# elisabeth96/nerf-rs

Hardware: AMD Instinct MI355X
Metric: rays/sec, lego 800x800 (64 coarse + 128 fine samples per ray) (higher is better)
Workload: dtype f32

## Files before the change

nerf-rs_amd/csrc/mlp_f32_core.hip.h:

```cpp
#pragma once
#include <hip/hip_runtime.h>
#include <stdint.h>

#include "mlp_common.hip.h"
#include "mlp_layout.h"

#ifndef NERF_DIAG_NO_BARRIER
#define NERF_DIAG_NO_BARRIER 0
#endif
#ifndef NERF_DIAG_NO_DMA
#define NERF_DIAG_NO_DMA 0
#endif
#ifndef NERF_DIAG_NO_LDS
#define NERF_DIAG_NO_LDS 0
#endif

namespace mlpf32 {

using namespace nerfmlp;
using namespace mlpdev;

constexpr int kReluGroup = 16;
constexpr int kLdsGroup = 1;

struct Pipe {
    const LDS_AS char *rd_base;
    const LDS_AS char *ring_lane;
    uint32_t rd_slot_off;
    f32x4 nx[2 * kLdsGroup];
    f32x4 cu[2 * kLdsGroup];
    uint32_t ring_addr;
    uint32_t wr_slot_off;
    uint32_t next_off;
    uint32_t stream_bytes;
    const char *gbase;
    const char *cur_src;
    uint32_t cur_dst;
    uint32_t lane16;
    uint64_t zs_off;
    uint32_t zs_exec;
    uint32_t zs_total;
};

__device__ __forceinline__ void pipe_zskip_init(Pipe &P, int zero_skip) {
    P.zs_off = zero_skip ? 0ull : ~0ull;
    P.zs_exec = 0;
    P.zs_total = 0;
}

__device__ __forceinline__ void pipe_zskip_report(const Pipe &P, unsigned long long *stats, int lane) {
    if (stats && lane == 0) {
        atomicAdd(stats, (unsigned long long)P.zs_exec);
        atomicAdd(stats + 1, (unsigned long long)P.zs_total);
    }
}

__device__ __forceinline__ void pipe_next_chunk(Pipe &P) {
    uint32_t off = P.next_off, slot = P.wr_slot_off;
    asm volatile("" : "+s"(off), "+s"(slot));
    P.cur_src = P.gbase + off;
    P.cur_dst = P.ring_addr + slot;
    off += kChunkBytes;
    P.next_off = (off == P.stream_bytes) ? 0u : off;
    slot += kChunkBytes;
    P.wr_slot_off = (slot == kRingSlots * kChunkBytes) ? 0u : slot;
    dma_set_dst(P.cur_dst);
}

__device__ __forceinline__ void pipe_issue_piece(Pipe &P, int i) {
#if !NERF_DIAG_NO_DMA
    glds_piece_m0(P.lane16, P.cur_src, i);
#else
    (void)P; (void)i;
#endif
}

__device__ __forceinline__ void pipe_issue(Pipe &P) {
    pipe_next_chunk(P);
#pragma unroll
    for (int i = 0; i < 4; ++i) pipe_issue_piece(P, i);
}

__device__ __forceinline__ void pipe_sync(Pipe &P) {
#if NERF_DIAG_NO_BARRIER
    asm volatile("s_waitcnt vmcnt(%0)" ::"n"(4 * (kRingSlots - 3)) : "memory");
#else
    asm volatile("s_waitcnt vmcnt(%0)\n\ts_barrier" ::"n"(4 * (kRingSlots - 3)) : "memory");
#endif
    pipe_next_chunk(P);
}

__device__ __forceinline__ void pipe_mid_step(Pipe &P, int ms) {
    if (ms >= 4) {
        __builtin_amdgcn_sched_barrier(0);
        pipe_issue_piece(P, ms - 4);
        __builtin_amdgcn_sched_barrier(0);
    }
}

__device__ __forceinline__ void pipe_prime(Pipe &P) {
#pragma unroll
    for (int j = 0; j < kLdsGroup; ++j) {
        P.nx[2 * j] = *(const LDS_AS f32x4 *)(P.rd_base + j * 2048);
        P.nx[2 * j + 1] = *(const LDS_AS f32x4 *)(P.rd_base + j * 2048 + 1024);
    }
}

__device__ __forceinline__ void pipe_restart(Pipe &P) {
    asm volatile("s_waitcnt vmcnt(0)\n\ts_barrier" ::: "memory");
    P.next_off = 0;
    P.wr_slot_off = 0;
#pragma unroll
    for (int c = 0; c < kRingSlots - 1; ++c) pipe_issue(P);
    asm volatile("s_waitcnt vmcnt(0)\n\ts_barrier" ::: "memory");
    P.rd_slot_off = 0;
    P.rd_base = P.ring_lane;
    pipe_prime(P);
}

__device__ __forceinline__ void pipe_advance(Pipe &P, int ms, f32x4 &a0, f32x4 &a1) {
    constexpr int LG = kLdsGroup;
    if (ms % LG == 0) {
#pragma unroll
        for (int j = 0; j < 2 * LG; ++j) P.cu[j] = P.nx[j];
        int nxt = ms + LG;
        if (nxt == 8) {
            uint32_t off = P.rd_slot_off + kChunkBytes;
            off = (off == kRingSlots * kChunkBytes) ? 0u : off;
            P.rd_slot_off = off;
            P.rd_base = P.ring_lane + off;
            nxt = 0;
        }
#pragma unroll
        for (int j = 0; j < LG; ++j) {
#if NERF_DIAG_NO_LDS
            asm volatile("" : "+v"(P.nx[2 * j]), "+v"(P.nx[2 * j + 1]));
#else
            P.nx[2 * j] = *(const LDS_AS f32x4 *)(P.rd_base + (nxt + j) * 2048);
            P.nx[2 * j + 1] = *(const LDS_AS f32x4 *)(P.rd_base + (nxt + j) * 2048 + 1024);
#endif
        }
        __builtin_amdgcn_sched_barrier(0);
    }
    a0 = P.cu[2 * (ms % LG)];
    a1 = P.cu[2 * (ms % LG) + 1];
}

#define MFMA(a, b, c) __builtin_amdgcn_mfma_f32_32x32x2f32((a), (b), (c), 0, 0, 0)

__device__ __forceinline__ uint64_t relu_live(float &b) {
    int bits = __builtin_bit_cast(int, b);
    asm volatile("" : "+v"(bits));
    b = __builtin_bit_cast(float, bits);
    return __builtin_amdgcn_ballot_w64(bits != 0);
}

template <int NT, bool RELU>
__device__ __forceinline__ void tile_steps(const f32x16 &in, f32x16 (&out)[NT], Pipe &P) {
    static_assert(NT == 8 || NT == 4, "NT");
    constexpr int G = RELU ? kReluGroup : 1;
    float bq[G];
    if constexpr (RELU) P.zs_total += 16;
    if constexpr (NT == 8) {
        uint64_t live[G];
#pragma unroll
        for (int r = 0; r < 16; ++r) {
            f32x4 a0, a1;
            if ((r & 7) == 4) pipe_sync(P);
            pipe_advance(P, r & 7, a0, a1);
            if (r % G == 0) {
#pragma unroll
                for (int g = 0; g < G; ++g) bq[g] = RELU ? relu(in[r + g]) : in[r + g];
                if constexpr (RELU) {
#pragma unroll
                    for (int g = 0; g < G; ++g) live[g] = relu_live(bq[g]) | P.zs_off;
                }
                if (G > 1) __builtin_amdgcn_sched_barrier(0);
            }
            const float b = bq[r % G];
            if constexpr (RELU) {
                pipe_mid_step(P, r & 7);
                if (live[r % G] != 0) {
                    ++P.zs_exec;
                    out[0] = MFMA(a0[0], b, out[0]); out[1] = MFMA(a0[1], b, out[1]);
                    out[2] = MFMA(a0[2], b, out[2]); out[3] = MFMA(a0[3], b, out[3]);
                    out[4] = MFMA(a1[0], b, out[4]); out[5] = MFMA(a1[1], b, out[5]);
                    out[6] = MFMA(a1[2], b, out[6]); out[7] = MFMA(a1[3], b, out[7]);
                }
            } else {
                out[0] = MFMA(a0[0], b, out[0]); out[1] = MFMA(a0[1], b, out[1]);
                pipe_mid_step(P, r & 7);
                out[2] = MFMA(a0[2], b, out[2]); out[3] = MFMA(a0[3], b, out[3]);
                out[4] = MFMA(a1[0], b, out[4]); out[5] = MFMA(a1[1], b, out[5]);
                out[6] = MFMA(a1[2], b, out[6]); out[7] = MFMA(a1[3], b, out[7]);
            }
        }
    } else {
        constexpr int G2 = G < 2 ? 2 : G;
        float bq2[G2];
        uint64_t live[G2];
#pragma unroll
        for (int r = 0; r < 16; r += 2) {
            f32x4 a0, a1;
            if (r / 2 == 4) pipe_sync(P);
            pipe_advance(P, r / 2, a0, a1);
            if (r % G2 == 0) {
#pragma unroll
                for (int g = 0; g < G2; ++g) bq2[g] = RELU ? relu(in[r + g]) : in[r + g];
                if constexpr (RELU) {
#pragma unroll
                    for (int g = 0; g < G2; ++g) live[g] = relu_live(bq2[g]) | P.zs_off;
                }
                if (G2 > 2) __builtin_amdgcn_sched_barrier(0);
            }
            const float b0 = bq2[r % G2], b1 = bq2[r % G2 + 1];
            if (!RELU || live[r % G2] != 0) {
                if constexpr (RELU) ++P.zs_exec;
                out[0] = MFMA(a0[0], b0, out[0]); out[1] = MFMA(a0[1], b0, out[1]);
                out[2] = MFMA(a0[2], b0, out[2]); out[3] = MFMA(a0[3], b0, out[3]);
            }
            pipe_mid_step(P, r / 2);
            if (!RELU || live[r % G2 + 1] != 0) {
                if constexpr (RELU) ++P.zs_exec;
                out[0] = MFMA(a1[0], b1, out[0]); out[1] = MFMA(a1[1], b1, out[1]);
                out[2] = MFMA(a1[2], b1, out[2]); out[3] = MFMA(a1[3], b1, out[3]);
            }
        }
    }
}

template <int NT>
__device__ __forceinline__ void load_bias(f32x16 (&out)[NT], const LDS_AS float *bias, int h) {
#pragma unroll
    for (int nt = 0; nt < NT; ++nt) {
        const LDS_AS f32x4 *b = (const LDS_AS f32x4 *)(bias + (nt * 2 + h) * 16);
#pragma unroll
        for (int q = 0; q < 4; ++q) {
            const f32x4 v = b[q];
            out[nt][4 * q + 0] = v[0]; out[nt][4 * q + 1] = v[1]; out[nt][4 * q + 2] = v[2]; out[nt][4 * q + 3] = v[3];
        }
    }
}

template <bool RELU>
__device__ __forceinline__ void hidden_layer(const f32x16 (&in)[8], f32x16 (&out)[8], const LDS_AS float *bias,
                                             Pipe &P, int h) {
    load_bias<8>(out, bias, h);
#pragma unroll
    for (int t = 0; t < 8; ++t) tile_steps<8, RELU>(in[t], out, P);
}

__device__ __forceinline__ float alpha_pre(const f32x16 (&Y)[8], const LDS_AS float *small, int h) {
    const LDS_AS f32x4 *w = (const LDS_AS f32x4 *)(small + kAlphaWOff + h * 128);
    float a0 = 0.f, a1 = 0.f, a2 = 0.f, a3 = 0.f;
#pragma unroll
    for (int t = 0; t < 8; ++t) {
#pragma unroll
        for (int q = 0; q < 4; ++q) {
            const f32x4 wv = w[t * 4 + q];
            a0 = fmaf(wv[0], relu(Y[t][4 * q + 0]), a0);
            a1 = fmaf(wv[1], relu(Y[t][4 * q + 1]), a1);
            a2 = fmaf(wv[2], relu(Y[t][4 * q + 2]), a2);
            a3 = fmaf(wv[3], relu(Y[t][4 * q + 3]), a3);
        }
    }
    return xhalf_sum((a0 + a1) + (a2 + a3)) + small[kMiscOff + 0];
}

__device__ __forceinline__ float alpha_head(const f32x16 (&Y)[8], const LDS_AS float *small, int h) { return fmaxf(alpha_pre(Y, small, h), 0.f); }

}
```

nerf-rs_amd/csrc/mlp_kernel.hip:

```cpp
#include <hip/hip_runtime.h>
#include <stdint.h>
#include <stdio.h>

#include "mlp_f32_core.hip.h"
#include "mlp_kernel.h"

using namespace nerfmlp;
using namespace mlpdev;

using namespace mlpf32;

template <bool FULL, int MODE>
__global__ __launch_bounds__(256, 1) void nerf_mlp_kernel(const MlpArgs A) {
    extern __shared__ __attribute__((aligned(16))) char smem[];
    const LDS_AS char *lds = (const LDS_AS char *)smem;
    const LDS_AS float *small = (const LDS_AS float *)(lds + kRingSlots * kChunkBytes);

    const int tid = threadIdx.x;
    const int lane = tid & 63;
    const int wave = __builtin_amdgcn_readfirstlane(tid >> 6);
    const int p = lane & 31;
    const int h = lane >> 5;
    const int lane16 = lane * 16;

    {
        float *dst = (float *)(smem + kRingSlots * kChunkBytes);
        for (int i = tid; i < kSmallFloats; i += 256) dst[i] = A.small_params[i];
    }

    Pipe P;
    P.lane16 = lane16;
    P.ring_lane = lds + lane16;
    P.ring_addr = (uint32_t)(uintptr_t)lds + wave * 4096;
    P.wr_slot_off = 0;
    P.next_off = 0;
    P.stream_bytes = (FULL ? kChunksFullFolded : kChunksSigma) * kChunkBytes;
    P.gbase = (const char *)A.wstream + wave * 4096;
    pipe_zskip_init(P, A.zero_skip);
    __syncthreads();
#pragma unroll
    for (int c = 0; c < kRingSlots - 1; ++c) pipe_issue(P);
    asm volatile("s_waitcnt vmcnt(0)\n\ts_barrier" ::: "memory");
    unsigned long long clk0 = 0, rt0 = 0;
    if (A.clock_out) { clk0 = __builtin_amdgcn_s_memtime(); rt0 = __builtin_amdgcn_s_memrealtime(); }
    P.rd_slot_off = 0;
    P.rd_base = P.ring_lane;
#pragma unroll
    for (int j = 0; j < kLdsGroup; ++j) {
        P.nx[2 * j] = *(const LDS_AS f32x4 *)(P.rd_base + j * 2048);
        P.nx[2 * j + 1] = *(const LDS_AS f32x4 *)(P.rd_base + j * 2048 + 1024);
    }

    const int n_points = MODE == MLP_MODE_LIST ? list_length(A) : A.n_points;
    const int n_tiles = (n_points + kPointsPerBlock - 1) / kPointsPerBlock;
    constexpr int LOAD = (!FULL && MODE == MLP_MODE_POINTS) ? 4 : MODE;
    constexpr bool ORDER = FULL && MODE == MLP_MODE_RAYS;
    const int order_tiles = ORDER ? A.order_tiles : 0, order_points = ORDER ? A.order_points : 0;
    const int lane_part = (MODE == MLP_MODE_RAYS && A.ray_map.wt.ss) ? wave_tile_lane_part(A.ray_map.wt, p) : p;
    auto ordered = [&](int T) { return ORDER && T < order_tiles; };
    auto map_tile = [&](int T) { return ORDER ? max(T - order_tiles, 0) : T; };
    auto base_of = [&](int T) {
        return MODE == MLP_MODE_RAYS ? order_points + ray_launch_base(A.ray_map, map_tile(T), wave) : T * kPointsPerBlock + wave * kPointsPerWave;
    };
    auto lane_of = [&](int T) { return (MODE == MLP_MODE_RAYS && ray_launch_tiled(A.ray_map, map_tile(T))) ? lane_part : p; };
    auto entry_of = [&](int T) {
        return ordered(T) ? (int)min(A.order_table[(size_t)T * kPointsPerBlock + wave * kPointsPerWave + p], (unsigned)order_points - 1u) : 0;
    };
    const int G = gridDim.x;
    TileWalk walk = {0, 0};
    auto next_round_tile = [&]() { return tile_walk_next(walk, (int)blockIdx.x, G, A.tile_rotation != 0); };
    int tile_next = next_round_tile();
    int tile_next2 = next_round_tile();
    int base_next = base_of(blockIdx.x);
    int ord_cur = entry_of(blockIdx.x), ord_next = entry_of(tile_next);
    RawIn nxt = load_raw_at<LOAD>(A, ordered(blockIdx.x) ? ord_cur : base_next + lane_of(blockIdx.x));
    for (int tile = blockIdx.x; tile < n_tiles; tile = tile_next, tile_next = tile_next2, tile_next2 = next_round_tile()) {
        const int slot = ordered(tile) ? ord_cur : base_next + lane_of(tile);
        const bool valid = slot < n_points;
        base_next = base_of(tile_next);
        if (ORDER) { ord_cur = ord_next; ord_next = entry_of(tile_next2); }
        const RawIn in = nxt;
        nxt = load_raw_at<LOAD>(A, ordered(tile_next) ? ord_cur : base_next + lane_of(tile_next));
        float px, py, pz;
        point_of<MODE>(A, in, px, py, pz);
        const float dx = in.dx, dy = in.dy, dz = in.dz;
        const unsigned entry = __builtin_bit_cast(unsigned, in.b);
        const size_t i = MODE == MLP_MODE_LIST ? (size_t)(entry & 0x7fffffffu) : (size_t)slot;
        const bool audit = MODE == MLP_MODE_LIST && (entry >> 31) != 0;

        f32x16 E[2];
        encode_point(px, py, pz, h, E);

        f32x16 X[8], Y[8];

        load_bias<8>(X, small + kBiasOff + 0 * 256, h);
        tile_steps<8, false>(E[0], X, P);
        tile_steps<8, false>(E[1], X, P);

        float sigma = 0.f;
        hidden_layer<true>(X, Y, small + kBiasOff + 1 * 256, P, h);
        hidden_layer<true>(Y, X, small + kBiasOff + 2 * 256, P, h);
        hidden_layer<true>(X, Y, small + kBiasOff + 3 * 256, P, h);
        hidden_layer<true>(Y, X, small + kBiasOff + 4 * 256, P, h);
        load_bias<8>(Y, small + kBiasOff + 5 * 256, h);
        tile_steps<8, false>(E[0], Y, P);
        tile_steps<8, false>(E[1], Y, P);
#pragma unroll
        for (int t = 0; t < 8; ++t) tile_steps<8, true>(X[t], Y, P);
        hidden_layer<true>(Y, X, small + kBiasOff + 6 * 256, P, h);
        hidden_layer<true>(X, Y, small + kBiasOff + 7 * 256, P, h);
        const float pre = alpha_pre(Y, small, h);
        sigma = fmaxf(pre, 0.f);
        if (MODE == MLP_MODE_GRID) {
            if (valid && h == 0 && A.sigma_out) A.sigma_out[i] = sigma;
            if (A.occ_bits) {
                const unsigned word = (unsigned)__ballot(valid && h == 0 && sigma > A.occ_threshold);
                const int slot0 = tile * kPointsPerBlock + wave * kPointsPerWave;
                if (lane == 0 && slot0 < n_points) A.occ_bits[slot0 >> 5] = word;
            }
        } else
        if (valid && h == 0) A.sigma_out[i] = audit ? pre : sigma;
        if (FULL && A.skip_empty) {
            LDS_AS int *vote = (LDS_AS int *)(lds + kRingSlots * kChunkBytes) + kMiscOff + 8;
            const bool any_wg = tile_has_density(vote, valid && sigma > 0.0f, wave, lane);
            if (!any_wg) {
                if (valid && h == 0) {
                    A.rgb_out[3 * (size_t)i + 0] = 0.f; A.rgb_out[3 * (size_t)i + 1] = 0.f; A.rgb_out[3 * (size_t)i + 2] = 0.f;
                }
                if (A.skip_counter && tid == 0) atomicAdd(A.skip_counter, 1ull);
                pipe_restart(P);
                continue;
            }
        }
        if (FULL) {
            f32x16 D;
            encode_dir(dx, dy, dz, h, D);
            f32x16 V[4];
            load_bias<4>(V, small + kBiasViewOff, h);
#pragma unroll
            for (int t = 0; t < 8; ++t) tile_steps<4, true>(Y[t], V, P);
            tile_steps<4, false>(D, V, P);
            float c[3];
            rgb_head(V, small, h, c);
            if (valid && h == 0) {
                A.rgb_out[3 * (size_t)i + 0] = c[0];
                A.rgb_out[3 * (size_t)i + 1] = c[1];
                A.rgb_out[3 * (size_t)i + 2] = c[2];
            }
        }
    }
    asm volatile("s_waitcnt vmcnt(0)" ::: "memory");
    pipe_zskip_report(P, A.zskip_stats, lane);
    if (A.clock_out && tid == 0) {
        A.clock_out[2 * blockIdx.x] = __builtin_amdgcn_s_memtime() - clk0;
        A.clock_out[2 * blockIdx.x + 1] = __builtin_amdgcn_s_memrealtime() - rt0;
    }
}

hipError_t nerf_zskip_clear(unsigned long long *stats, hipStream_t stream) {
    return stats ? hipMemsetAsync(stats, 0, 2 * sizeof(unsigned long long), stream) : hipSuccess;
}
hipError_t nerf_zskip_print(const char *what, unsigned long long *stats, hipStream_t stream) {
    if (!stats) return hipSuccess;
    unsigned long long h[2] = {0, 0};
    hipError_t e = hipMemcpyAsync(h, stats, sizeof h, hipMemcpyDeviceToHost, stream);
    if (e == hipSuccess) e = hipStreamSynchronize(stream);
    if (e == hipSuccess) fprintf(stderr, "nerf zskip: %s relu_ksteps_executed=%llu relu_ksteps_total=%llu\n", what, h[0], h[1]);
    return e;
}

template <bool FULL, int MODE>
static hipError_t launch_t(const MlpArgs &a, int n_blocks, hipStream_t stream) {
    hipError_t e = nerf_zskip_clear(a.zskip_stats, stream);
    if (e != hipSuccess) return e;
    hipLaunchKernelGGL((nerf_mlp_kernel<FULL, MODE>), dim3(n_blocks), dim3(256), kLdsBytes, stream, a);
    e = hipGetLastError();
    if (e != hipSuccess) return e;
    static const char *const modes[4] = {"points", "rays", "list", "grid"};
    char what[48];
    snprintf(what, sizeof what, "nerf_mlp_kernel<%s,%s>", FULL ? "full" : "sigma", modes[MODE]);
    return nerf_zskip_print(what, a.zskip_stats, stream);
}

hipError_t nerf_mlp_init() {
    const void *ks[7] = {(const void *)nerf_mlp_kernel<true, MLP_MODE_POINTS>, (const void *)nerf_mlp_kernel<true, MLP_MODE_RAYS>,
                         (const void *)nerf_mlp_kernel<false, MLP_MODE_RAYS>, (const void *)nerf_mlp_kernel<true, MLP_MODE_LIST>,
                         (const void *)nerf_mlp_kernel<false, MLP_MODE_LIST>, (const void *)nerf_mlp_kernel<false, MLP_MODE_POINTS>,
                         (const void *)nerf_mlp_kernel<false, MLP_MODE_GRID>};
    for (int i = 0; i < 7; ++i) {
        hipError_t e = hipFuncSetAttribute(ks[i], hipFuncAttributeMaxDynamicSharedMemorySize, kLdsBytes);
        if (e != hipSuccess) return e;
    }
    return hipSuccess;
}

static hipError_t launch_mlp_rays(const MlpArgs &a, bool full, int n_blocks, hipStream_t stream) {
    MlpArgs g = a;
    DepthOrder d = {0, 0, 0, 0};
    if (a.order_table) d = nerf_mlp_depth_order(a, full);
    g.order_tiles = d.tiles; g.order_points = d.points;
    if (!d.tiles) g.order_table = nullptr;
    g.ray_map = ray_launch_map_of(a.n_points - d.points, a.samples_per_ray, a.rays_per_row, full, a.ray_grouping != 0, a.wave_tiling != 0);
    return full ? launch_t<true, MLP_MODE_RAYS>(g, n_blocks, stream) : launch_t<false, MLP_MODE_RAYS>(g, n_blocks, stream);
}

hipError_t nerf_mlp_launch(const MlpArgs &a, bool full, int n_blocks, hipStream_t stream) {
    if (a.n_points <= 0) return hipSuccess;
    const int n_tiles = (a.n_points + kPointsPerBlock - 1) / kPointsPerBlock;
    if (n_blocks > n_tiles) n_blocks = n_tiles;
    if (n_blocks < 1) n_blocks = 1;
    if (a.mode == MLP_MODE_LIST) {
        if (!a.point_list || !a.point_list_count) return hipErrorInvalidValue;
        return full ? launch_t<true, MLP_MODE_LIST>(a, n_blocks, stream) : launch_t<false, MLP_MODE_LIST>(a, n_blocks, stream);
    }
    if (a.mode == MLP_MODE_GRID) {
        if (full || a.grid_n[0] <= 0 || a.grid_n[1] <= 0 || a.grid_n[2] <= 0 || (!a.sigma_out && !a.occ_bits)) return hipErrorInvalidValue;
        const unsigned long long plane = (unsigned long long)a.grid_n[0] * (unsigned long long)a.grid_n[1];
        if (plane > (unsigned long long)a.n_points || plane * (unsigned long long)a.grid_n[2] != (unsigned long long)a.n_points) return hipErrorInvalidValue;
        return launch_t<false, MLP_MODE_GRID>(a, n_blocks, stream);
    }
    if (a.mode == MLP_MODE_POINTS)
        return full ? launch_t<true, MLP_MODE_POINTS>(a, n_blocks, stream) : launch_t<false, MLP_MODE_POINTS>(a, n_blocks, stream);
    return launch_mlp_rays(a, full, n_blocks, stream);
}
```

nerf-rs_amd/csrc/mlp_kernel_seq.hip:

```cpp
#include <hip/hip_runtime.h>
#include <stdint.h>

#include "mlp_f32_core.hip.h"
#include "mlp_kernel.h"
#include "mlp_seq_common.hip.h"

using namespace nerfmlp;
using namespace mlpdev;
using namespace mlpf32;
using namespace mlpseq;

namespace {

__device__ __forceinline__ void pipe_start(Pipe &P, const LDS_AS char *lds, int lane16, int wave, const char *stream, int n_chunks) {
    P.lane16 = lane16;
    P.ring_lane = lds + lane16;
    P.ring_addr = (uint32_t)(uintptr_t)lds + wave * 4096;
    P.wr_slot_off = 0;
    P.next_off = 0;
    P.stream_bytes = n_chunks * kChunkBytes;
    P.gbase = stream + wave * 4096;
    __syncthreads();
#pragma unroll
    for (int c = 0; c < kRingSlots - 1; ++c) pipe_issue(P);
    asm volatile("s_waitcnt vmcnt(0)\n\ts_barrier" ::: "memory");
    P.rd_slot_off = 0;
    P.rd_base = P.ring_lane;
    pipe_prime(P);
}

}

constexpr int kStageTiles = 3;
constexpr int kStageCols = kStageTiles * 32;
constexpr int kStageTileBytes = 32 * 1024;
constexpr int kStageOff = kLdsBytes;
constexpr int kStageMetaOff = kStageOff + kStageTiles * kStageTileBytes;
constexpr int kStageVoteOff = kStageMetaOff + kStageCols * 16;
constexpr int kSeqLdsBytes = kStageVoteOff + 16;
static_assert(kSeqLdsBytes <= 160 * 1024, "LDS");
constexpr int kColourChunks = kChunksColourFolded;
static_assert(kRingSlots == 3, "the colour passes keep all three ring slots in flight");

namespace {

__device__ __forceinline__ void ring_issue_start(Pipe &P, const char *gbase, uint32_t stream_bytes, int n_chunks) {
    P.gbase = gbase;
    P.stream_bytes = stream_bytes;
    P.next_off = 0;
    P.wr_slot_off = 0;
    for (int c = 0; c < n_chunks; ++c) pipe_issue(P);
    P.rd_slot_off = 0;
    P.rd_base = P.ring_lane;
}

__device__ __forceinline__ void ring_advance(Pipe &P) {
    uint32_t off = P.rd_slot_off + kChunkBytes;
    off = (off == kRingSlots * kChunkBytes) ? 0u : off;
    P.rd_slot_off = off;
    P.rd_base = P.ring_lane + off;
}

__device__ __forceinline__ bool colour_sync(Pipe &P, int chunk, bool last_pass, const char *trunk_gbase) {
    if (last_pass && chunk == kColourChunks - 3) { P.gbase = trunk_gbase; P.stream_bytes = kChunksSigma * kChunkBytes; P.next_off = 0; }
    asm volatile("s_waitcnt vmcnt(4) lgkmcnt(0)\n\ts_barrier" ::: "memory");
    const bool refill = !(last_pass && chunk == kColourChunks - 1);
    if (refill) pipe_next_chunk(P);
    return refill;
}

struct Stage {
    LDS_AS char *tiles;
    LDS_AS f32x4 *meta;
    int head;
    int count;
};

__device__ __forceinline__ void load_b_tile(f32x4 (&raw)[4], const LDS_AS char *tile_lane, int tt) {
#pragma unroll
    for (int q = 0; q < 4; ++q) raw[q] = *(const LDS_AS f32x4 *)(tile_lane + (tt * 4 + q) * 1024);
}

__device__ __forceinline__ void bias_tile(f32x16 &acc, const LDS_AS float *bias_nt_h) {
    const LDS_AS f32x4 *b = (const LDS_AS f32x4 *)bias_nt_h;
#pragma unroll
    for (int q = 0; q < 4; ++q) { const f32x4 u = b[q]; acc[4 * q + 0] = u[0]; acc[4 * q + 1] = u[1]; acc[4 * q + 2] = u[2]; acc[4 * q + 3] = u[3]; }
}

__device__ __forceinline__ void store_tile(LDS_AS char *tile, int lane, int slot_t, const f32x16 &acc) {
#pragma unroll
    for (int q = 0; q < 4; ++q) {
        f32x4 u;
        u[0] = acc[4 * q + 0]; u[1] = acc[4 * q + 1]; u[2] = acc[4 * q + 2]; u[3] = acc[4 * q + 3];
        *(LDS_AS f32x4 *)(tile + lane * 16 + (slot_t * 4 + q) * 1024) = u;
    }
}

__device__ __forceinline__ void colour_pass(Pipe &P, const Stage &S, int n_cols, bool last_pass, const char *trunk_gbase, const SeqArgs &A,
                                            const LDS_AS float *small, int wave, int lane) {
    const int p = lane & 31, h = lane >> 5;
    const int t0 = S.head, t1 = S.head + 1 == kStageTiles ? 0 : S.head + 1;
    LDS_AS char *tile0 = S.tiles + t0 * kStageTileBytes, *tile1 = S.tiles + t1 * kStageTileBytes;
    const LDS_AS char *tl0 = tile0 + lane * 16, *tl1 = tile1 + lane * 16;
    const f32x4 m0 = S.meta[t0 * 32 + p], m1 = S.meta[t1 * 32 + p];

    const int v_off = wave * 4;
    float c_cur[16], c_nxt[16];
#pragma unroll
    for (int j = 0; j < 16; ++j) c_cur[j] = *(const LDS_AS float *)(P.rd_base + j * 1024 + v_off);
    f32x4 bn0[4], bn1[4];
    load_b_tile(bn0, tl0, 0);
    load_b_tile(bn1, tl1, 0);
    f32x16 V0, V1;
    bias_tile(V0, small + kBiasViewOff + (wave * 2 + h) * 16);
    V1 = V0;
    f32x16 D0, D1;
    encode_dir(m0[1], m0[2], m0[3], h, D0);
    encode_dir(m1[1], m1[2], m1[3], h, D1);
    int chunk = 0;
    for (int tt = 0; tt < 9; ++tt, ++chunk) {
        float bq0[16], bq1[16];
        if (tt < 8) {
#pragma unroll
            for (int q = 0; q < 4; ++q)
#pragma unroll
                for (int e = 0; e < 4; ++e) { bq0[4 * q + e] = relu(bn0[q][e]); bq1[4 * q + e] = relu(bn1[q][e]); }
        } else {
#pragma unroll
            for (int r = 0; r < 16; ++r) { bq0[r] = D0[r]; bq1[r] = D1[r]; }
        }
        __builtin_amdgcn_sched_barrier(0);
        bool refill = false;
#pragma unroll
        for (int j = 0; j < 16; ++j) {
            if (j == 8) {
                refill = colour_sync(P, chunk, last_pass, trunk_gbase);
                ring_advance(P);
                if (tt < 8) {
#pragma unroll
                    for (int k = 0; k < 16; ++k) c_nxt[k] = *(const LDS_AS float *)(P.rd_base + k * 1024 + v_off);
                    if (tt < 7) { load_b_tile(bn0, tl0, tt + 1); load_b_tile(bn1, tl1, tt + 1); }
                }
                __builtin_amdgcn_sched_barrier(0);
            }
            V0 = MFMA(c_cur[j], bq0[j], V0);
            if (j >= 8 && (j & 1) == 0) { __builtin_amdgcn_sched_barrier(0); if (refill) pipe_issue_piece(P, (j - 8) >> 1); __builtin_amdgcn_sched_barrier(0); }
            V1 = MFMA(c_cur[j], bq1[j], V1);
        }
#pragma unroll
        for (int k = 0; k < 16; ++k) c_cur[k] = c_nxt[k];
    }
    asm volatile("s_waitcnt lgkmcnt(0)\n\ts_barrier" ::: "memory");
    store_tile(tile0, lane, wave, V0);
    store_tile(tile1, lane, wave, V1);
    asm volatile("s_waitcnt lgkmcnt(0)\n\ts_barrier" ::: "memory");
    f32x16 VV0[4], VV1[4];
    if (wave < 3) {
#pragma unroll
        for (int t = 0; t < 4; ++t)
#pragma unroll
            for (int q = 0; q < 4; ++q) {
                const f32x4 u = *(const LDS_AS f32x4 *)(tl0 + (t * 4 + q) * 1024), v = *(const LDS_AS f32x4 *)(tl1 + (t * 4 + q) * 1024);
                VV0[t][4 * q + 0] = u[0]; VV0[t][4 * q + 1] = u[1]; VV0[t][4 * q + 2] = u[2]; VV0[t][4 * q + 3] = u[3];
                VV1[t][4 * q + 0] = v[0]; VV1[t][4 * q + 1] = v[1]; VV1[t][4 * q + 2] = v[2]; VV1[t][4 * q + 3] = v[3];
            }
    }
    asm volatile("s_waitcnt lgkmcnt(0)\n\ts_barrier" ::: "memory");
    if (wave < 3) {
        const float c0 = rgb_channel(VV0, small, h, wave), c1 = rgb_channel(VV1, small, h, wave);
        if (h == 0 && p < n_cols) A.rgb_out[3 * (size_t)__builtin_bit_cast(unsigned, m0[0]) + wave] = c0;
        if (h == 0 && 32 + p < n_cols) A.rgb_out[3 * (size_t)__builtin_bit_cast(unsigned, m1[0]) + wave] = c1;
    }
}

}

template <bool EXPORT>
__global__ __launch_bounds__(256, 1) void nerf_trunk_seq_kernel(const SeqArgs A) {
    extern __shared__ __attribute__((aligned(16))) char smem[];
    const LDS_AS char *lds = (const LDS_AS char *)smem;
    const LDS_AS float *small = (const LDS_AS float *)(lds + kRingSlots * kChunkBytes);
    LDS_AS int *vote = (LDS_AS int *)(lds + kRingSlots * kChunkBytes) + kMiscOff + 8;

    const int tid = threadIdx.x;
    const int lane = tid & 63;
    const int wave = __builtin_amdgcn_readfirstlane(tid >> 6);
    const int p = lane & 31;
    const int h = lane >> 5;
    {
        float *dst = (float *)(smem + kRingSlots * kChunkBytes);
        for (int i = tid; i < kSmallFloats; i += 256) dst[i] = A.small_params[i];
    }
    const char *trunk_gbase = (const char *)A.wstream + wave * 4096;
    const char *colour_gbase = trunk_gbase + (size_t)kChunksSigma * kChunkBytes;
    Pipe P;
    pipe_start(P, lds, lane * 16, wave, (const char *)A.wstream, kChunksSigma);
    pipe_zskip_init(P, A.zero_skip);

    Stage S;
    S.tiles = (LDS_AS char *)smem + kStageOff;
    S.meta = (LDS_AS f32x4 *)((LDS_AS char *)smem + kStageMetaOff);
    S.head = 0; S.count = 0;
    LDS_AS int *nlive = (LDS_AS int *)((LDS_AS char *)smem + kStageVoteOff);

    RayWork W;
    work_init(W, A);
    for (;;) {
        const bool running = work_acquire(W, A, vote, wave, lane);
        if (!running && !(EXPORT && S.count > 0)) break;
        ChunkIn c{};
        LiveInfo li{};
        f32x16 Y[8];
        if (running) {
            c = chunk_inputs(W, A, p);
            f32x16 E[2];
            encode_point(c.px, c.py, c.pz, h, E);
            f32x16 X[8];
            load_bias<8>(X, small + kBiasOff + 0 * 256, h);
            tile_steps<8, false>(E[0], X, P);
            tile_steps<8, false>(E[1], X, P);
            hidden_layer<true>(X, Y, small + kBiasOff + 1 * 256, P, h);
            hidden_layer<true>(Y, X, small + kBiasOff + 2 * 256, P, h);
            hidden_layer<true>(X, Y, small + kBiasOff + 3 * 256, P, h);
            hidden_layer<true>(Y, X, small + kBiasOff + 4 * 256, P, h);
            load_bias<8>(Y, small + kBiasOff + 5 * 256, h);
            tile_steps<8, false>(E[0], Y, P);
            tile_steps<8, false>(E[1], Y, P);
#pragma unroll
            for (int tt = 0; tt < 8; ++tt) tile_steps<8, true>(X[tt], Y, P);
            hidden_layer<true>(Y, X, small + kBiasOff + 6 * 256, P, h);
            hidden_layer<true>(X, Y, small + kBiasOff + 7 * 256, P, h);
            const float sigma = alpha_head(Y, small, h);
            li = chunk_scan(W, A, c, sigma, p, h);
        }
        if (EXPORT) {
            if (running) {
                if (lane == 0) nlive[wave] = li.n_live;
                W.live_done += (unsigned)li.n_live;
            }
            asm volatile("s_waitcnt vmcnt(0) lgkmcnt(0)\n\ts_barrier" ::: "memory");
            int n_w4[4] = {0, 0, 0, 0};
            if (running) {
#pragma unroll
                for (int w = 0; w < 4; ++w) n_w4[w] = __builtin_amdgcn_readfirstlane(nlive[w]);
            }
            const int total = n_w4[0] + n_w4[1] + n_w4[2] + n_w4[3];
            int ring = 0;
            if (S.count + total >= 64 || (!running && S.count > 0)) {
                ring_issue_start(P, colour_gbase, kColourChunks * kChunkBytes, 3);
                ring = 1;
            }
            for (int w = 0; w <= 4; ++w) {
                const int n_w = w == 0 ? n_w4[0] : w == 1 ? n_w4[1] : w == 2 ? n_w4[2] : w == 3 ? n_w4[3] : 0;
                const bool flush = w < 4 ? (S.count + n_w > kStageCols) : (S.count >= 64 || (!running && S.count > 0));
                if (flush) {
                    if (ring == 1) asm volatile("s_waitcnt vmcnt(8) lgkmcnt(0)\n\ts_barrier" ::: "memory");
                    else asm volatile("s_waitcnt lgkmcnt(0)\n\ts_barrier" ::: "memory");
                    ring = 2;
                    while (S.count >= 64 || (!running && S.count > 0)) {
                        const int n_cols = S.count < 64 ? S.count : 64;
                        const int rest = S.count - n_cols;
                        const bool last = !(rest >= 64 || (!running && rest > 0)) && w == 4 && running;
                        colour_pass(P, S, n_cols, last, trunk_gbase, A, small, wave, lane);
                        S.head = (S.head + (n_cols > 32 ? 2 : 1)) % kStageTiles;
                        S.count = rest;
                        if (last) { ring = 0; pipe_prime(P); }
                    }
                }
                if (w < 4 && wave == w && li.live) {
                    int slot = S.head * 32 + S.count + __popcll(li.mask & ((1ull << p) - 1ull));
                    slot = slot >= kStageCols ? slot - kStageCols : slot;
                    LDS_AS char *dst = S.tiles + (slot >> 5) * kStageTileBytes + ((slot & 31) + 32 * h) * 16;
#pragma unroll
                    for (int tt = 0; tt < 8; ++tt)
#pragma unroll
                        for (int q = 0; q < 4; ++q) {
                            f32x4 v;
                            v[0] = Y[tt][4 * q + 0]; v[1] = Y[tt][4 * q + 1]; v[2] = Y[tt][4 * q + 2]; v[3] = Y[tt][4 * q + 3];
                            *(LDS_AS f32x4 *)(dst + (tt * 4 + q) * 1024) = v;
                        }
                    if (h == 0) {
                        f32x4 m;
                        m[0] = __builtin_bit_cast(float, (unsigned)(c.base + c.s)); m[1] = c.dx; m[2] = c.dy; m[3] = c.dz;
                        S.meta[slot] = m;
                    }
                }
                S.count += n_w;
            }
            if (ring != 0) {
                asm volatile("s_waitcnt vmcnt(0) lgkmcnt(0)\n\ts_barrier" ::: "memory");
                ring_issue_start(P, trunk_gbase, kChunksSigma * kChunkBytes, kRingSlots - 1);
                asm volatile("s_waitcnt vmcnt(0)\n\ts_barrier" ::: "memory");
                pipe_prime(P);
            }
        }
        if (!running) break;
        chunk_advance(W, A, c, li.cut, p, h);
    }
    asm volatile("s_waitcnt vmcnt(0)" ::: "memory");
    work_done(W, A, lane);
    pipe_zskip_report(P, A.zskip_stats, lane);
}

hipError_t nerf_seq_init() {
    hipError_t e = hipFuncSetAttribute((const void *)nerf_trunk_seq_kernel<true>, hipFuncAttributeMaxDynamicSharedMemorySize, kSeqLdsBytes);
    if (e != hipSuccess) return e;
    return hipFuncSetAttribute((const void *)nerf_trunk_seq_kernel<false>, hipFuncAttributeMaxDynamicSharedMemorySize, kLdsBytes);
}

size_t nerf_seq_h8_bytes(size_t n_samples) {
    const size_t tiles = (n_samples + kPointsPerBlock - 1) / kPointsPerBlock * kWavesPerBlock;
    return tiles * kH8TileFloats * sizeof(float);
}

hipError_t nerf_trunk_seq_launch(const SeqArgs &a, bool export_live, int n_blocks, hipStream_t stream) {
    if (a.n_rays <= 0 || a.samples_per_ray <= 0) return hipSuccess;
    n_blocks = trunk_blocks(a, n_blocks);
    if (export_live && !a.rgb_out) return hipErrorInvalidValue;
    hipError_t e = nerf_zskip_clear(a.zskip_stats, stream);
    if (e != hipSuccess) return e;
    if (export_live) hipLaunchKernelGGL(nerf_trunk_seq_kernel<true>, dim3(n_blocks), dim3(256), kSeqLdsBytes, stream, a);
    else hipLaunchKernelGGL(nerf_trunk_seq_kernel<false>, dim3(n_blocks), dim3(256), kLdsBytes, stream, a);
    e = hipGetLastError();
    if (e != hipSuccess) return e;
    return nerf_zskip_print(export_live ? "nerf_trunk_seq_kernel<export>" : "nerf_trunk_seq_kernel<sigma>", a.zskip_stats, stream);
}
```

Measured before the change: 773,700.

## Deepen LDS weight-fragment prefetch to a three-step look-ahead register ring

Replaces the single-step next/current LDS fragment double buffer with a four-entry register ring that reads weight fragments three MFMA steps ahead. pipe_sync gains an lgkmcnt bound so LDS reads belonging to the current chunk can stay in flight across the barrier. The aim is to hide LDS read latency behind more MFMA work, at the cost of extra VGPRs and tighter correctness reasoning about which reads are in flight at the ring-slot barrier. The seq kernel also re-materialises the lane indices p and h through an opaque asm each loop iteration, apparently to shape register allocation.

```diff
diff --git a/nerf-rs_amd/csrc/mlp_f32_core.hip.h b/nerf-rs_amd/csrc/mlp_f32_core.hip.h
--- a/nerf-rs_amd/csrc/mlp_f32_core.hip.h
+++ b/nerf-rs_amd/csrc/mlp_f32_core.hip.h
@@ -21,14 +21,15 @@
 using namespace mlpdev;
 
 constexpr int kReluGroup = 16;
-constexpr int kLdsGroup = 1;
+constexpr int kALook = 3;
+constexpr int kARing = kALook + 1;
+static_assert(8 % kARing == 0 && kALook < 8 - 4, "ring phase / the look-ahead must not reach past the chunk pipe_sync has proven landed");
 
 struct Pipe {
     const LDS_AS char *rd_base;
     const LDS_AS char *ring_lane;
     uint32_t rd_slot_off;
-    f32x4 nx[2 * kLdsGroup];
-    f32x4 cu[2 * kLdsGroup];
+    f32x4 ar[2 * kARing];
     uint32_t ring_addr;
     uint32_t wr_slot_off;
     uint32_t next_off;
@@ -82,10 +83,12 @@
 }
 
 __device__ __forceinline__ void pipe_sync(Pipe &P) {
+    constexpr int kLgkmBound = 4 * kALook;
+    static_assert(kLgkmBound <= 15 && kLgkmBound <= 2 * (4 + kALook), "lgkmcnt bound: the reads it leaves in flight must all be of chunk c");
 #if NERF_DIAG_NO_BARRIER
-    asm volatile("s_waitcnt vmcnt(%0)" ::"n"(4 * (kRingSlots - 3)) : "memory");
+    asm volatile("s_waitcnt vmcnt(%0) lgkmcnt(%1)" ::"n"(4 * (kRingSlots - 3)), "n"(kLgkmBound) : "memory");
 #else
-    asm volatile("s_waitcnt vmcnt(%0)\n\ts_barrier" ::"n"(4 * (kRingSlots - 3)) : "memory");
+    asm volatile("s_waitcnt vmcnt(%0) lgkmcnt(%1)\n\ts_barrier" ::"n"(4 * (kRingSlots - 3)), "n"(kLgkmBound) : "memory");
 #endif
     pipe_next_chunk(P);
 }
@@ -100,9 +103,9 @@
 
 __device__ __forceinline__ void pipe_prime(Pipe &P) {
 #pragma unroll
-    for (int j = 0; j < kLdsGroup; ++j) {
-        P.nx[2 * j] = *(const LDS_AS f32x4 *)(P.rd_base + j * 2048);
-        P.nx[2 * j + 1] = *(const LDS_AS f32x4 *)(P.rd_base + j * 2048 + 1024);
+    for (int j = 0; j < kALook; ++j) {
+        P.ar[2 * j] = *(const LDS_AS f32x4 *)(P.rd_base + j * 2048);
+        P.ar[2 * j + 1] = *(const LDS_AS f32x4 *)(P.rd_base + j * 2048 + 1024);
     }
 }
 
@@ -119,31 +122,24 @@
 }
 
 __device__ __forceinline__ void pipe_advance(Pipe &P, int ms, f32x4 &a0, f32x4 &a1) {
-    constexpr int LG = kLdsGroup;
-    if (ms % LG == 0) {
-#pragma unroll
-        for (int j = 0; j < 2 * LG; ++j) P.cu[j] = P.nx[j];
-        int nxt = ms + LG;
-        if (nxt == 8) {
-            uint32_t off = P.rd_slot_off + kChunkBytes;
-            off = (off == kRingSlots * kChunkBytes) ? 0u : off;
-            P.rd_slot_off = off;
-            P.rd_base = P.ring_lane + off;
-            nxt = 0;
-        }
-#pragma unroll
-        for (int j = 0; j < LG; ++j) {
+    int nxt = ms + kALook;
+    if (nxt == 8) {
+        uint32_t off = P.rd_slot_off + kChunkBytes;
+        off = (off == kRingSlots * kChunkBytes) ? 0u : off;
+        P.rd_slot_off = off;
+        P.rd_base = P.ring_lane + off;
+    }
+    nxt &= 7;
+    const int in = (ms + kALook) % kARing, cur = ms % kARing;
 #if NERF_DIAG_NO_LDS
-            asm volatile("" : "+v"(P.nx[2 * j]), "+v"(P.nx[2 * j + 1]));
+    asm volatile("" : "+v"(P.ar[2 * in]), "+v"(P.ar[2 * in + 1]));
 #else
-            P.nx[2 * j] = *(const LDS_AS f32x4 *)(P.rd_base + (nxt + j) * 2048);
-            P.nx[2 * j + 1] = *(const LDS_AS f32x4 *)(P.rd_base + (nxt + j) * 2048 + 1024);
-#endif
-        }
-        __builtin_amdgcn_sched_barrier(0);
-    }
-    a0 = P.cu[2 * (ms % LG)];
-    a1 = P.cu[2 * (ms % LG) + 1];
+    P.ar[2 * in] = *(const LDS_AS f32x4 *)(P.rd_base + nxt * 2048);
+    P.ar[2 * in + 1] = *(const LDS_AS f32x4 *)(P.rd_base + nxt * 2048 + 1024);
+#endif
+    __builtin_amdgcn_sched_barrier(0);
+    a0 = P.ar[2 * cur];
+    a1 = P.ar[2 * cur + 1];
 }
 
 #define MFMA(a, b, c) __builtin_amdgcn_mfma_f32_32x32x2f32((a), (b), (c), 0, 0, 0)
diff --git a/nerf-rs_amd/csrc/mlp_kernel.hip b/nerf-rs_amd/csrc/mlp_kernel.hip
--- a/nerf-rs_amd/csrc/mlp_kernel.hip
+++ b/nerf-rs_amd/csrc/mlp_kernel.hip
@@ -46,9 +46,9 @@
     P.rd_slot_off = 0;
     P.rd_base = P.ring_lane;
 #pragma unroll
-    for (int j = 0; j < kLdsGroup; ++j) {
-        P.nx[2 * j] = *(const LDS_AS f32x4 *)(P.rd_base + j * 2048);
-        P.nx[2 * j + 1] = *(const LDS_AS f32x4 *)(P.rd_base + j * 2048 + 1024);
+    for (int j = 0; j < kALook; ++j) {
+        P.ar[2 * j] = *(const LDS_AS f32x4 *)(P.rd_base + j * 2048);
+        P.ar[2 * j + 1] = *(const LDS_AS f32x4 *)(P.rd_base + j * 2048 + 1024);
     }
 
     const int n_points = MODE == MLP_MODE_LIST ? list_length(A) : A.n_points;
diff --git a/nerf-rs_amd/csrc/mlp_kernel_seq.hip b/nerf-rs_amd/csrc/mlp_kernel_seq.hip
--- a/nerf-rs_amd/csrc/mlp_kernel_seq.hip
+++ b/nerf-rs_amd/csrc/mlp_kernel_seq.hip
@@ -185,8 +185,8 @@
     const int tid = threadIdx.x;
     const int lane = tid & 63;
     const int wave = __builtin_amdgcn_readfirstlane(tid >> 6);
-    const int p = lane & 31;
-    const int h = lane >> 5;
+    const int p_lane = lane & 31;
+    const int h_lane = lane >> 5;
     {
         float *dst = (float *)(smem + kRingSlots * kChunkBytes);
         for (int i = tid; i < kSmallFloats; i += 256) dst[i] = A.small_params[i];
@@ -206,6 +206,8 @@
     RayWork W;
     work_init(W, A);
     for (;;) {
+        int p = p_lane, h = h_lane;
+        asm volatile("" : "+v"(p), "+v"(h));
         const bool running = work_acquire(W, A, vote, wave, lane);
         if (!running && !(EXPORT && S.count > 0)) break;
         ChunkIn c{};
```

New measurement: 776,000 (median of 3 runs). Within noise of the previous version (+0.3%).
